# proycon/analiticcl

Hardware: AMD Instinct MI355X
Metric: scored (query,candidate) pairs/sec + queries/sec, 200k-lexicon, len≤16, 1/2/4/8 GPU (higher is better)
Workload: dtype u8

## Files before the change

### analiticcl_amd/csrc/engine.hip

```cpp
#include <hip/hip_runtime.h>

#include <algorithm>
#include <atomic>
#include <functional>
#include <chrono>
#include <cmath>
#include <cstdio>
#include <cstdlib>
#include <cstring>
#include <map>
#include <memory>
#include <mutex>
#include <unordered_map>
#include <numeric>
#include <thread>
#include <type_traits>

#include "engine_internal.h"

namespace anx {

#define HIP_TRY(expr)                                                                          \
  do {                                                                                         \
    hipError_t _e = (expr);                                                                    \
// ... 1043 lines not shown
}
void kernel_timer_enable(bool on) {
  KTimer& t = ktimer();
  std::lock_guard<std::mutex> lk(t.mu);
  ktimer_resolve_locked(t);
  t.acc.clear();
  t.on.store(on);
}
bool kernel_timer_read(const char* name, double* total_ms, uint64_t* launches) {
  KTimer& t = ktimer();
  std::lock_guard<std::mutex> lk(t.mu);
  ktimer_resolve_locked(t);
  auto it = t.acc.find(name ? name : "");
  if (it == t.acc.end()) { if (total_ms) *total_ms = 0.0; if (launches) *launches = 0; return false; }
  if (total_ms) *total_ms = it->second.first;
  if (launches) *launches = it->second.second;
  return true;
}

#include "launch_plan.hpp"

template <int NP>
static void launch_scan(ScanArgs A, uint32_t nadj, uint32_t nbits, uint32_t nsad, hipStream_t st, hipEvent_t e0, hipEvent_t e1) {
  (void)hipEventRecord(e0, st);
  const bool gen = A.want_exact || A.qpairs || !A.drop_len;
  if (nadj) {
    A.ntiles = nadj;
    if (gen) hipLaunchKernelGGL((k_scan_adj<true>), dim3((nadj + 3) / 4), dim3(256), 0, st, A);
    else hipLaunchKernelGGL((k_scan_adj<false>), dim3((nadj + 3) / 4), dim3(256), 0, st, A);
    A.tiles += nadj;
    nbits -= nadj;
  }
  if (nbits) {
    A.ntiles = nbits;
    if (A.want_exact || A.qpairs || !A.drop_len) hipLaunchKernelGGL((k_scan_bits<true>), dim3((nbits + 3) / 4), dim3(256), 0, st, A);
    else hipLaunchKernelGGL((k_scan_bits<false>), dim3((nbits + 3) / 4), dim3(256), 0, st, A);
  }
  (void)hipEventRecord(e1, st);
  if (nsad) {
    A.tiles += nbits;
    A.ntiles = nsad;
    hipLaunchKernelGGL((k_scan_sad<NP>), dim3((nsad + 3) / 4), dim3(256), 0, st, A);
  }
}

static int ensure_raw(Batch* b, size_t slots_per_region, std::string& err) {
  uint32_t shift = 10;
  while (((size_t)1 << shift) < slots_per_region) ++shift;
  if (shift > 25) { err = "pair list exceeds 2^31 slots: split the batch"; return ANX_ELIMIT; }
  const size_t cap = (size_t)SCAN_REGIONS << shift;
  if (cap <= b->raw_cap) return ANX_OK;
  for (void* p : {(void*)b->raw, (void*)b->p_score, (void*)b->p_meta})
    if (p) pool_free(p);
  b->raw = nullptr; b->p_score = nullptr; b->p_meta = nullptr; b->raw_cap = 0;
  int rc;
  if ((rc = dalloc(&b->raw, cap, err))) return rc;
  b->raw_cap = cap;
  b->region_shift = shift;
  return ANX_OK;
}
static int ensure_pair_outputs(Batch* b, std::string& err) {
  if (b->p_meta) return ANX_OK;
  int rc;
  if ((rc = dalloc(&b->p_score, b->raw_cap, err)) || (rc = dalloc(&b->p_meta, b->raw_cap, err))) return rc;
  return ANX_OK;
}
// ... 109 lines not shown

int Run::setup() {
  int rc;
  hints_apply(dl, b);
  if (b->raw_cap == 0 && b->hinted && (rc = ensure_raw(b, (size_t)b->prev_maxfill + (b->prev_maxfill >> 3) + 4096, err))) return rc;
  if (b->raw_cap == 0 && (rc = ensure_raw(b, (nq * (size_t)140 + (size_t)b->ntiles * SCAN_CHUNK) / SCAN_REGIONS / cap_div() + 4096, err)))
    return rc;
  region_cap = 1u << b->region_shift;
  fill_cap = b->prev_maxfill ? (uint32_t)std::min<size_t>(region_cap, (size_t)b->prev_maxfill + (b->prev_maxfill >> 3) + FS_BLK) : region_cap;
  b->fill_cap_launched = fill_cap;
  HIP_TRY(hipEventRecord(b->ev[0], st));
  return ANX_OK;
}

int Run::scan() {
  int rc;
  HIP_TRY(hipMemsetAsync(b->ctl, 0, HR_N * sizeof(uint32_t), st));
  if (b->ntiles == 0) { HIP_TRY(hipEventRecord(b->ev_scan0, st)); HIP_TRY(hipEventRecord(b->ev[5], st)); }
  if (b->ntiles) {
    ScanArgs A = scan_args_of(dl);
    A.tiles = b->d_tiles; A.ntiles = b->ntiles; A.q_bits = b->q_bits; A.q_cv = b->q_cv;
    A.chunk = SCAN_CHUNK;
    A.chunk_fused = switches().scan_chunk_fused ? (uint32_t)switches().scan_chunk_fused : SCAN_CHUNK_FUSED;
#ifdef ANX_DEBUG_SWITCHES
    { const char* e = getenv("ANX_SCAN_CHUNK"); const int v = e ? atoi(e) : 0; if (v >= 32 && v <= 1024) A.chunk = (uint32_t)v; }
#endif
    A.raw = b->raw; A.region_cap = region_cap; A.rctr = b->rctr; A.qexact = b->qexact; A.want_exact = stop;
    A.drop_len = (!stop && !b->keep_all_pairs) ? 1 : 0;
    A.q_rec = b->q_rec;
    A.fuse = (switches().fuse_prefilter && switches().prefilter && A.drop_len) ? 1 : 0;
    A.qpairs = nullptr;
    if (b->count_pairs) {
      if (!b->qpairs && (rc = dalloc(&b->qpairs, nq, err))) return rc;
      HIP_TRY(hipMemsetAsync(b->qpairs, 0, nq * sizeof(uint32_t), st));
      A.qpairs = b->qpairs;
    }
    A.dbg = 0;
#ifdef ANX_DEBUG_SWITCHES
    { const char* e = getenv("ANX_SCAN_DBG"); A.dbg = e ? atoi(e) : 0; }
#endif
    const uint32_t nsad = b->n_sad_tiles, nbits = A.ntiles - nsad, nadj = std::min(b->n_adj_tiles, nbits);
    with_nplanes(dl->nplanes, [&](auto np) { launch_scan<decltype(np)::value>(A, nadj, nbits, nsad, st, b->ev_scan0, b->ev[5]); });
  }
  HIP_TRY(hipEventRecord(b->ev[1], st));
  b->n_raw = (uint32_t)(SCAN_REGIONS << b->region_shift);
  return ANX_OK;
// ... 171 lines not shown
    maxfill = std::max(maxfill, c[RC_RAW]);
    b->region_fill[r] = c[RC_RAW];
    n_slots += c[RC_RAW];
    n_valid += c[RC_VALID];
    n_fused += c[RC_FUSED];
    n_adj_rows += c[RC_ADJ];
    n_adj_rows_first += c[RC_ADJ_FIRST];
    for (int i = 0; i <= NBITPLANES; ++i) {
      uint64_t v;
      memcpy(&v, c + RC_TESTS + 2 * i, sizeof v);
      b->n_tests_kind[i] += v;
      b->n_class_tests += v;
    }
    surv_fill = std::max(surv_fill, h[HR_SCTR + r * RC_STRIDE]);
    nsel += h[HR_SCTR + r * RC_STRIDE + 1];
    for (int l = 0; l < 3; ++l) list_fill = std::max(list_fill, h[HR_LCTR + (l * SCAN_REGIONS + r) * RC_STRIDE]);
  }
  const uint32_t total_surv = h[HR_TOTAL_SURV], total_results = h[HR_TOTAL_RESULTS];
  b->conf_fallback = b->conf_mode != 0 && (h[HR_CONF + 1] != 0 || b->conf_skipped);
  b->stats.n_conf_scripts = b->conf_mode ? h[HR_CONF] : 0;
  b->stats.n_adj_tiles = std::min(b->n_adj_tiles, b->ntiles - b->n_sad_tiles);
  int rc;
  bool again = false;
  if (maxfill > (1u << b->region_shift)) {
    if ((rc = ensure_raw(b, (size_t)maxfill + (maxfill >> 3) + 4096, err))) return rc;
    again = true;
  }
  if (maxfill > b->fill_cap_launched) again = true;
  if ((size_t)surv_fill > b->surv_region_cap) again = true;
  if (list_fill && (size_t)list_fill > b->list_cap) again = true;
  if (!dl->any_variants && (size_t)total_surv > b->surv_cap) {
    if ((rc = ensure_surv(b, (size_t)total_surv + (total_surv >> 2) + 1024, err))) return rc;
    again = true;
  }
  b->prev_maxfill = std::max(b->prev_maxfill, maxfill);
  b->prev_surv_fill = std::max(b->prev_surv_fill, surv_fill);
  b->prev_list_fill = std::max(b->prev_list_fill, list_fill);
  if (again) { *retry = true; b->runs_finished++; return ANX_OK; }
  if (b->runs_finished++ == 0) hints_record(dl, b, maxfill, surv_fill, list_fill, total_surv);
  if (maxfill == 0) b->n_raw = 0;
  b->n_pairs = n_valid - h[HR_CTR + CTR_SKIPPED];
  b->n_surv = total_surv;
  b->n_sel = nsel;
  b->n_results = total_results;
  b->max_rows = h[HR_CTR + CTR_MAXROWS];
  b->ran = true;
  anx_batch_stats& s = b->stats;
  s.n_queries = nq;
  s.n_pairs = b->n_pairs;
  s.n_class_tests = b->n_class_tests;
  s.n_results = total_results;
  s.n_scan_blocks = b->ntiles;
  for (int i = 0; i <= NBITPLANES; ++i) s.n_tests_kind[i] = b->n_tests_kind[i];
  s.n_pair_slots = n_slots;
  s.n_survivors = total_surv;
// ... 656 lines not shown
```

### analiticcl_amd/csrc/host_model.cpp

```cpp
#include "host_model.h"
#include "adjacency.h"

#include <sched.h>
#if defined(__SSE2__)
#include <emmintrin.h>
#endif

#include <thread>

#include <algorithm>
#include <cmath>
#include <cstdio>
#include <cstring>
#include <fstream>
#include <functional>
#include <numeric>
#include <sstream>

#include "unicode_tables.inc"

namespace anx {

static std::vector<uint32_t> make_primes() {
  std::vector<uint32_t> p;
// ... 482 lines not shown
  lexicons.push_back(path);
  return ANX_OK;
}

static int pick_planes(int nsym) {
  const int need = (nsym + 3) / 4;
  for (int v : {8, 16, 24, 32, 42})
    if (need <= v) return v;
  return -1;
}

namespace {
struct SwitchDef { const char* name; void (*set)(Switches&, const char*); };
int flag01(const char* v, int dflt) { return !v ? dflt : (v[0] == '0' ? 0 : 1); }
const SwitchDef kSwitches[] = {
    {"ANX_ENCODE", [](Switches& s, const char* v) { s.encode_host = v && strcmp(v, "host") == 0; }},
    {"ANX_SCAN", [](Switches& s, const char* v) { s.scan_sad = v && strcmp(v, "sad") == 0; }},
    {"ANX_SCAN_WALK", [](Switches& s, const char* v) { s.scan_walk_flat = v && strcmp(v, "flat") == 0; }},
    {"ANX_SCAN_TQ", [](Switches& s, const char* v) { const int x = v ? atoi(v) : 0; s.scan_tq = x >= 1 && x <= 64 ? x : 0; }},
    {"ANX_SCAN_ADJ", [](Switches& s, const char* v) { s.scan_adj = flag01(v, 1); }},
    {"ANX_ADJ_BUILD", [](Switches& s, const char* v) { s.adj_build_host = v && strcmp(v, "host") == 0; }},
    {"ANX_ADJ_CLOSURE", [](Switches& s, const char* v) { const int x = v ? atoi(v) : 2; s.adj_closure = x >= 0 && x <= kAdjMaxClosure ? x : kAdjMaxClosure; }},
    {"ANX_SCAN_CHUNK_FUSED", [](Switches& s, const char* v) { const int x = v ? atoi(v) : 0; s.scan_chunk_fused = x >= 32 && x <= 1024 ? x : 0; }},
    {"ANX_ADJ_FAIL", [](Switches& s, const char* v) { s.adj_fail = flag01(v, 0); }},
    {"ANX_SMALL", [](Switches& s, const char* v) { s.small_path = flag01(v, 1); }},
    {"ANX_SURV_SEG", [](Switches& s, const char* v) { const int x = v ? atoi(v) : 32; s.surv_seg = x >= 0 && x <= 256 ? x : 32; }},
    {"ANX_ENC_PRIORITY", [](Switches& s, const char* v) { s.enc_priority = flag01(v, 1); }},
    {"ANX_HINTS", [](Switches& s, const char* v) { s.hints = flag01(v, 1); }},
    {"ANX_ADJ_MB", [](Switches& s, const char* v) { const long x = v ? atol(v) : 0; s.adj_budget_mb = x > 0 ? x : 16384; }},
    {"ANX_SIG_GROUPS", [](Switches& s, const char* v) { const int x = v ? atoi(v) : 0; s.sig_groups = x >= 1 && x <= 8 ? x : 0; }},
    {"ANX_SIG_SEARCH", [](Switches& s, const char* v) { s.sig_search = flag01(v, 1); }},
    {"ANX_PREFILTER", [](Switches& s, const char* v) { s.prefilter = flag01(v, 1); }},
    {"ANX_SCORE_FAST", [](Switches& s, const char* v) { s.score_fast = flag01(v, 1); }},
    {"ANX_FS_SPLIT", [](Switches& s, const char* v) { s.fs_split = flag01(v, 1); }},
    {"ANX_FS_PLANES", [](Switches& s, const char* v) { s.fs_planes = flag01(v, 1); }},
    {"ANX_FS_B7", [](Switches& s, const char* v) { s.fs_b7 = flag01(v, 1); }},
    {"ANX_SCAN_FUSE", [](Switches& s, const char* v) { s.fuse_prefilter = flag01(v, 1); }},
    {"ANX_CAP_DIV", [](Switches& s, const char* v) { const long x = v ? atol(v) : 0; s.cap_div = x > 1 ? x : 1; }},
    {"ANX_MAX_BATCH", [](Switches& s, const char* v) { const long x = v ? atol(v) : 0; s.max_batch = x > 0 ? x : (4l << 20); }},
    {"ANX_RUN_OVERLAP", [](Switches& s, const char* v) { s.run_overlap = (v && atoi(v) == 0 && v[0] == '0') ? 0 : 1; }},
    {"ANX_SHARD_POLICY", [](Switches& s, const char* v) { s.shard_by_length = (v && strcmp(v, "range") == 0) ? 0 : 1; }},
    {"ANX_SHARD_MIN", [](Switches& s, const char* v) { const long x = v ? atol(v) : 0; s.shard_min = x > 0 ? x : 8192; }},
    {"ANX_CONFUSABLES", [](Switches& s, const char* v) { s.confusables_host = v && strcmp(v, "host") == 0; }},
    {"ANX_LATTICE", [](Switches& s, const char* v) { s.lattice_host = v && strcmp(v, "host") == 0; }},
    {"ANX_SEARCH_ONEPASS", [](Switches& s, const char* v) { s.search_onepass = flag01(v, 1); }},
    {"ANX_ENCODE_TIMING", [](Switches& s, const char* v) { s.encode_timing = v != nullptr && v[0] != 0 && v[0] != '0'; }},
// ... 524 lines not shown
```

### analiticcl_amd/csrc/host_model.h

```cpp
#pragma once
#include <functional>
#include <cstdint>
#include <atomic>
#include <memory>
#include <mutex>
#include <string>
#include <unordered_map>
#include <vector>

#include "../../include/anx.h"
#include "confusables_core.hpp"
#include "contextrules_flat.hpp"

namespace anx {

constexpr int kMaxSymbols = 255;
constexpr int kMaxAlphabet = 166;
constexpr int kMaxAnagramDistance = 12;
constexpr int kMaxEditDistance = 12;

struct AlphabetMember {
  std::string bytes;
  int nchars;
};
// ... 32 lines not shown
  int scan_walk_flat = 0;
  int scan_tq = 0;
  int scan_adj = 1;
  int adj_build_host = 0;
  int adj_closure = 2;
  long adj_budget_mb = 16384;
  int sig_groups = 0;
  int sig_search = 1;
  int prefilter = 1;
  int score_fast = 1;
  int fs_planes = 1;
  int fs_split = 1;
  int fs_b7 = 1;
  int fuse_prefilter = 1;
  long cap_div = 1;
  long max_batch = 4l << 20;
  int run_overlap = 1;
  int shard_by_length = 1;
  long shard_min = 8192;
  int confusables_host = 0;
  int lattice_host = 0;
  int search_onepass = 1;
  int scan_chunk_fused = 0;
  int adj_fail = 0;
  int small_path = 1;
  int enc_priority = 1;
  int hints = 1;
  int encode_timing = 0;
  int search_timing = 0;
  int search_parts = 4;
  long search_parts_min = 2l << 20;
  long search_part_bytes = 4l << 20;
  int search_prio = 1;
  int search_early_output = 1;
  int search_first_pct = 50;
  int surv_seg = 32;
  int learn_fold_host = 0;
  int learn_hash_bits = 63;
};
Switches& switches();
bool set_switch(const char* name, const char* value);

struct VariantRef {
  bool variant_of;
  uint64_t id;
  double score;
// ... 178 lines not shown
```

### analiticcl_amd/csrc/kernels_common.hpp

```cpp
#pragma once

struct Tile {
  uint32_t q0, nq;
  uint32_t s0, s1;
  uint32_t k;
  uint32_t lq;
  uint32_t sig_lo, sig_hi;
  uint32_t kind;
  uint32_t d;
  uint32_t kend;
  uint32_t ball0, balln;
  uint32_t adj;
  uint32_t flags;
};
constexpr uint32_t BALL_MAX = 4096;
constexpr uint32_t SIG_BYTE_MAX = 120;

constexpr int kSymbolPlanesMaxA = 61;
__host__ __device__ inline void symbol_planes16(const uint8_t* row, uint32_t len, uint32_t (&w)[3]) {
  uint32_t p[6] = {0u, 0u, 0u, 0u, 0u, 0u};
  for (uint32_t i = 0; i < 16u && i < len; ++i) {
    const uint32_t v = (uint32_t)row[i] + 1u;
    for (uint32_t b = 0; b < 6u; ++b) p[b] |= ((v >> b) & 1u) << i;
  }
  w[0] = p[0] | p[1] << 16; w[1] = p[2] | p[3] << 16; w[2] = p[4] | p[5] << 16;
}

constexpr int NBITPLANES = 4;
constexpr uint32_t SCAN_TQ = 64;
constexpr uint32_t SCAN_TQ_DEFAULT = 48;
constexpr uint32_t SCAN_HITS = 512;
constexpr uint32_t SCAN_MASKW = 2048;
constexpr uint32_t SCAN_PBUF = 128;
constexpr uint32_t SCAN_CHUNK = 256;
constexpr uint32_t SCAN_CHUNK_FUSED = 128;
constexpr uint32_t SCAN_REGIONS = 64;
constexpr uint32_t RC_STRIDE = 32;
constexpr uint32_t RAW_INVALID = 0xFFFFFFFFu;
constexpr uint32_t RAW_ENTRY_MASK = 0x3FFFFFFFu;
constexpr uint32_t RAW_PREFILTERED = 0x40000000u;
constexpr uint32_t META_SKIPPED = 0xFFFFFFFFu;

struct EntRec {
  uint32_t vocab, freq, order, meta;
};

struct DevAlphabet {
  int16_t* fast = nullptr;
  uint32_t* coff = nullptr;
  uint4* cand = nullptr;
  uint8_t* bytes = nullptr;
  uint8_t* sym_group = nullptr;
  uint2* lower = nullptr;
  uint32_t nlower = 0;
  uint32_t* siglen_begin = nullptr;
};

struct BatchShell {
// ... 191 lines not shown
```

### analiticcl_amd/csrc/kernels_scan.hpp

```cpp
#pragma once

enum { RC_RAW = 0, RC_VALID = 1, RC_FUSED = 2 , RC_TESTS = 4 ,
       RC_ADJ = 14 , RC_ADJ_FIRST = 15  };

struct WaveOut {
  uint32_t base, left;
  uint32_t emitted;
  uint32_t nbase;
  uint32_t split;
  uint32_t rbase, rend;
  uint32_t* ctr;
  uint32_t chunk;
};
__device__ inline uint32_t wave_inclusive_scan(uint32_t x) {
  uint32_t v = x;
  v += (uint32_t)__builtin_amdgcn_update_dpp(0, (int)x, 0x111, 0xF, 0xF, false);
  v += (uint32_t)__builtin_amdgcn_update_dpp(0, (int)x, 0x112, 0xF, 0xF, false);
  v += (uint32_t)__builtin_amdgcn_update_dpp(0, (int)x, 0x113, 0xF, 0xF, false);
  v += (uint32_t)__builtin_amdgcn_update_dpp(0, (int)v, 0x114, 0xF, 0xE, false);
  v += (uint32_t)__builtin_amdgcn_update_dpp(0, (int)v, 0x118, 0xF, 0xC, false);
  v += (uint32_t)__builtin_amdgcn_update_dpp(0, (int)v, 0x142, 0xA, 0xF, false);
  v += (uint32_t)__builtin_amdgcn_update_dpp(0, (int)v, 0x143, 0xC, 0xF, false);
  return v;
}
__device__ inline uint32_t wave_reserve(WaveOut& w, uint32_t ntot, uint32_t lane, uint32_t* total_out) {
  const uint32_t incl = wave_inclusive_scan(ntot);
  const uint32_t total = (uint32_t)__builtin_amdgcn_readlane((int)incl, 63);
  *total_out = total;
  w.split = w.left;
  if (total > w.left) {
    const uint32_t rest = total - w.left;
    const uint32_t need = rest > w.chunk ? rest : w.chunk;
    uint32_t b = 0;
    if (lane == 0) b = atomicAdd(&w.ctr[RC_RAW], need);
    w.nbase = w.rbase + __shfl(b, 0);
  }
  return incl - ntot;
}
__device__ inline void wave_reserve_total(WaveOut& w, uint32_t total, uint32_t lane) {
  w.split = w.left;
  if (total > w.left) {
    const uint32_t rest = total - w.left;
    const uint32_t need = rest > w.chunk ? rest : w.chunk;
    uint32_t b = 0;
    if (lane == 0) b = atomicAdd(&w.ctr[RC_RAW], need);
    w.nbase = w.rbase + (uint32_t)__builtin_amdgcn_readfirstlane((int)b);
  }
}
__device__ inline uint32_t wave_slot(const WaveOut& w, uint32_t g) {
  return g < w.split ? w.base + g : w.nbase + (g - w.split);
}
__device__ inline void wave_commit(WaveOut& w, uint32_t total) {
  if (total > w.left) {
    const uint32_t rest = total - w.left;
    const uint32_t need = rest > w.chunk ? rest : w.chunk;
    w.base = w.nbase + rest;
    w.left = need - rest;
  } else {
    w.base += total;
    w.left -= total;
  }
  w.emitted += total;
}
__device__ inline void wave_close(const WaveOut& w, uint32_t lane, uint2* __restrict__ raw) {
  for (uint32_t i = lane; i < w.left; i += 64)
    if (w.base + i < w.rend) raw[w.base + i] = make_uint2(RAW_INVALID, 0u);
  if (lane == 0 && w.emitted) atomicAdd(&w.ctr[RC_VALID], w.emitted);
}

struct ScanArgs {
  const Tile* tiles;
  uint32_t ntiles;
  const uint32_t* q_bits;
  const uint32_t* q_cv;
  const uint32_t* cls_bits;
  const uint32_t* cls_planes;
  const uint4* scan_rec;
  const uint2* scan_rec34;
  uint32_t pad_rec;
  uint32_t cstride;
  uint32_t pad_class;
  const uint8_t* cls_len;
  const uint32_t* cls_off;
  const uint4* sig;
  const uint4* sig_e;
  const uint4* sighash;
  const uint4* sighash_e;
  uint32_t hash_mask;
  const unsigned long long* ball;
  const uint32_t* adj_hdr;
  const uint2* adj_planes;
  const uint32_t* adj_ids;
  const uint32_t* sig_cbeg;
  uint2* raw;
  uint32_t region_cap;
  uint32_t chunk;
  uint32_t chunk_fused;
  uint32_t* rctr;
  const uint32_t* qexact;
  int want_exact;
  int drop_len;
  const uint4* q_rec;
  const uint4* e_rec;
  int fuse;
  uint32_t* qpairs;
  int dbg;
};

__device__ inline int32_t bcnt_acc(uint32_t x, int32_t acc) {
  int32_t r;
  asm("v_bcnt_u32_b32 %0, %1, %2" : "=v"(r) : "v"(x), "v"(acc));
  return r;
}
__device__ inline int32_t bcnt_acc_s(uint32_t x, int32_t acc) {
  int32_t r;
  asm("v_bcnt_u32_b32 %0, %1, %2" : "=v"(r) : "v"(x), "s"(acc));
  return r;
}

template <bool BITS, int NP, bool GEN, bool ADJ = false>
__device__ inline void scan_tile(const ScanArgs& AA, const Tile& t, uint32_t item, uint32_t* __restrict__ stage, uint32_t* __restrict__ hits,
                                 uint32_t* __restrict__ qlds, uint4* __restrict__ qsym, uint32_t* __restrict__ pbuf) {
  ScanArgs A = AA;
  if (!GEN) { A.want_exact = 0; A.qpairs = nullptr; A.drop_len = 1; A.qexact = nullptr; }
  constexpr int CPL = BITS ? 4 : (NP <= 8 ? 4 : NP <= 16 ? 2 : 1);
  constexpr int W = BITS ? NBITPLANES : NP;
  constexpr int QSTRIDE = BITS ? NBITPLANES : NP;
  constexpr uint32_t CHUNK = 64u * CPL;
  const uint32_t lane = threadIdx.x & 63;
  const uint32_t* __restrict__ cls_words = BITS ? A.cls_bits : A.cls_planes;
  const uint8_t* __restrict__ cls_len = A.cls_len;
  const uint32_t* __restrict__ cls_off = A.cls_off;
  uint2* __restrict__ raw = A.raw;
  const uint32_t cstride = A.cstride;
  const uint32_t region = item % SCAN_REGIONS;
  WaveOut wo{0, 0, 0, 0, 0, region * A.region_cap, (region + 1) * A.region_cap, A.rctr + region * RC_STRIDE, A.chunk};
  uint32_t ns = 0;
  uint32_t nchunks = 0;
  uint32_t arend = 0;
  int32_t alc[4] = {0, 0, 0, 0};
  uint2 apl[4] = {};
  uint32_t aid[4] = {};
  auto adj_load = [&](uint32_t row, uint2 (&pl)[4], uint32_t (&id)[4]) {
#pragma unroll
    for (int j = 0; j < 4; ++j) {
      pl[j] = make_uint2(0u, 0u);
      id[j] = A.pad_rec;
      if (row + (uint32_t)j < arend) {
        const size_t p = (size_t)(row + (uint32_t)j) * 64u + lane;
        pl[j] = A.adj_planes[p];
        id[j] = A.adj_ids[p];
      }
    }
  };
  {
    const uint32_t* __restrict__ src = (BITS ? A.q_bits : A.q_cv) + (size_t)t.q0 * QSTRIDE;
    for (uint32_t i = lane; i < t.nq * QSTRIDE; i += 64) qlds[i] = src[i];
  }
  const bool fuse = BITS && A.fuse && t.lq <= 16u && t.d <= 3u;
  if (fuse) wo.chunk = A.chunk_fused;
  if (BITS && fuse && lane < t.nq) qsym[lane] = rec32(A.q_rec, t.q0 + lane)[0];
  constexpr uint32_t PBUF = SCAN_PBUF;
  uint32_t nfused = 0;
  uint32_t npb = 0, phead = 0;

  uint32_t nhits = 0;
  uint32_t counted_only = 0;
  auto emit_dense = [&](bool fin) {
    while (npb >= 64u || (fin && npb)) {
      const uint32_t cnt = npb < 64u ? npb : 64u;
      const bool act = lane < cnt;
      const uint32_t pr = pbuf[(phead + lane) & (PBUF - 1u)];
      const uint32_t e = act ? (pr & 0x3FFFFFFu) : 0u, ql = act ? (pr >> 26) : 0u;
      bool keep = act;
      uint32_t flag = 0u;
      if (ANX_DBG(A.dbg) & 16) keep = false;
      if (BITS && fuse && !(ANX_DBG(A.dbg) & 16)) {
        nfused += cnt;
        const uint4 C = rec32(A.e_rec, e)[0];
        const int lc = (int)(rec32(A.e_rec, e)[1].x & 0xFFu), lq = (int)t.lq, d = (int)t.d;
        const uint4 Q = qsym[ql];
        const bool filt = act && lc <= 16;
        const int ml = lq > lc ? lq : lc;
// ... 18 lines not shown
      if (total) {
        wave_reserve_total(wo, total, lane);
        if (keep) {
          const uint32_t q = t.q0 + ql;
          uint32_t exact = 0u;
          if (A.want_exact) exact = A.qexact[q] == A.scan_rec[e].w ? 0x80000000u : 0u;
          const uint32_t g = __builtin_amdgcn_mbcnt_hi((uint32_t)(km >> 32), __builtin_amdgcn_mbcnt_lo((uint32_t)km, 0u));
          const uint32_t pos = wave_slot(wo, g);
          if (pos < wo.rend) raw[pos] = make_uint2(q, e | exact | flag);
        }
        wave_commit(wo, total);
      }
      phead = (phead + cnt) & (PBUF - 1u);
      npb -= cnt;
    }
  };
  auto flush = [&]() {
    for (uint32_t r0 = 0; r0 < nhits; r0 += 64) {
      const uint32_t idx = r0 + lane;
      uint32_t c = 0, m = 0, e0 = 0, ne = 0, qb = 0;
      if (idx < nhits) {
        bool count_only;
        if (BITS) {
          const uint32_t hx = reinterpret_cast<const uint16_t*>(hits + SCAN_HITS)[idx];
          m = hits[idx];
          qb = ((hx >> 8) & 1u) << 5;
          count_only = (hx >> 9) & 1u;
          e0 = stage[hx & 0xFFu];
          ne = 1;
          c = A.qpairs ? A.scan_rec[e0].w : 0u;
        } else {
          c = hits[2 * idx];
          m = hits[2 * idx + 1];
          qb = ((c >> 27) & 1u) << 5;
          c &= (1u << 27) - 1u;
          const uint32_t lc = cls_len[c];
          e0 = cls_off[c];
          ne = cls_off[c + 1] - e0;
          const uint32_t diff = lc > t.lq ? lc - t.lq : t.lq - lc;
          count_only = A.drop_len && diff > t.d;
        }
        if (A.qpairs) {
          for (uint32_t mm = m; mm; mm &= mm - 1u) {
            const uint32_t q = t.q0 + qb + (uint32_t)__ffs((int)mm) - 1u;
            if (!A.want_exact || A.qexact[q] == 0xFFFFFFFFu || A.qexact[q] == c) atomicAdd(&A.qpairs[q], ne);
          }
        }
        if (count_only) {
          counted_only += (uint32_t)__popc(m) * ne;
          m = 0;
        }
// ... 22 lines not shown
          m &= m - 1u;
          const uint32_t q = t.q0 + qb + bit;
          const uint32_t exact = (A.want_exact && A.qexact[q] == c) ? 0x80000000u : 0u;
          for (uint32_t i = 0; i < ne; ++i, ++g) dst[g] = make_uint2(q, (e0 + i) | exact);
        }
      } else {
        while (m) {
          const uint32_t bit = (uint32_t)__ffs((int)m) - 1u;
          m &= m - 1u;
          const uint32_t q = t.q0 + qb + bit;
          const uint32_t exact = (A.want_exact && A.qexact[q] == c) ? 0x80000000u : 0u;
          for (uint32_t i = 0; i < ne; ++i, ++g) {
            const uint32_t pos = wave_slot(wo, g);
            if (pos < wo.rend) raw[pos] = make_uint2(q, (e0 + i) | exact);
          }
        }
      }
      wave_commit(wo, total);
    }
    nhits = 0;
  };

  auto process = [&]() {
    ++nchunks;
    if (ANX_DBG(A.dbg) & 2) return;
    uint32_t cid[CPL], cw[CPL][W];
    int32_t thr[CPL];
    const bool need34 = BITS && ((t.kend >> 8) & 0xFFu) < t.nq;
#pragma unroll
    for (int j = 0; j < CPL; ++j) {
      const uint32_t idx = (uint32_t)j * 64u + lane;
      int32_t lc;
      if (ADJ) {
        const uint2 pl = apl[j];
        const uint32_t id = aid[j];
        stage[idx] = id;
        uint2 hi = make_uint2(0u, 0u);
        if (need34) hi = A.scan_rec34[id];
        cw[j][0] = pl.x; cw[j][1] = pl.y;
        if (W > 2) { cw[j][2] = hi.x; cw[j][W - 1] = hi.y; }
        lc = alc[j];
        const int32_t diff = lc > (int32_t)t.lq ? lc - (int32_t)t.lq : (int32_t)t.lq - lc;
        cid[j] = (A.drop_len && diff > (int32_t)t.d) ? id | (1u << 28) : id;
      } else {
      cid[j] = idx < ns ? stage[idx] : (BITS ? A.pad_rec : A.pad_class);
      if (BITS) {
        const uint4 mt = A.scan_rec[cid[j]];
        uint2 hi = make_uint2(0u, 0u);
        if (need34) hi = A.scan_rec34[cid[j]];
        const uint32_t plw[4] = {mt.x, mt.y, hi.x, hi.y};
#pragma unroll
        for (int p = 0; p < W; ++p) cw[j][p] = plw[p];
        lc = (int32_t)mt.z;
        const int32_t diff = lc > (int32_t)t.lq ? lc - (int32_t)t.lq : (int32_t)t.lq - lc;
        if (A.drop_len && diff > (int32_t)t.d) cid[j] |= 1u << 28;
      } else {
#pragma unroll
        for (int p = 0; p < W; ++p) cw[j][p] = cls_words[(size_t)p * cstride + cid[j]];
        lc = (int32_t)cls_len[cid[j]];
      }
      }
      if (BITS) {
        const int32_t need = ((int32_t)t.lq - (int32_t)t.k + lc + 1) >> 1;
        thr[j] = -(need < 1 ? 1 : need);
      } else {
// ... 31 lines not shown
        uint32_t qi = lo;
        for (; qi + 2 <= hi; qi += 2) {
          test_query(tw, qi);
          test_query(tw, qi + 1);
        }
        if (qi < hi) test_query(tw, qi);
      };
      if (BITS) {
        const uint32_t pend = qb + npass;
        auto clampr = [&](uint32_t x) { return (x < qb ? qb : (x > pend ? pend : x)) - qb; };
        const uint32_t b1 = clampr(t.kend & 0xFFu), b2 = clampr((t.kend >> 8) & 0xFFu), b3 = clampr((t.kend >> 16) & 0xFFu);
        run_queries(std::integral_constant<int, 1>{}, 0u, b1);
        run_queries(std::integral_constant<int, 2>{}, b1, b2);
        run_queries(std::integral_constant<int, 3>{}, b2, b3);
        run_queries(std::integral_constant<int, BITS ? 4 : 1>{}, b3, npass);
      } else {
        run_queries(std::integral_constant<int, BITS ? 1 : NP>{}, 0u, npass);
      }
      const uint32_t valid = npass >= 32u ? 0xFFFFFFFFu : ((1u << npass) - 1u);
      uint32_t any = 0;
#pragma unroll
      for (int j = 0; j < CPL; ++j) {
        hm[j] = ~hm[j] & valid;
        any |= hm[j];
      }
      if (__ballot(any != 0) == 0ull || (ANX_DBG(A.dbg) & 8)) continue;
#pragma unroll
      for (int j = 0; j < CPL; ++j) {
        const bool nz = hm[j] != 0;
        const unsigned long long bm = __ballot(nz);
        const uint32_t cnt = (uint32_t)__popcll(bm);
        if (cnt) {
          if (nz) {
            const uint32_t pos = nhits + __builtin_amdgcn_mbcnt_hi((uint32_t)(bm >> 32), __builtin_amdgcn_mbcnt_lo((uint32_t)bm, 0u));
            const uint32_t hmask = __brev(hm[j]) >> (32u - npass);
            if (BITS) {
              hits[pos] = hmask;
              reinterpret_cast<uint16_t*>(hits + SCAN_HITS)[pos] = (uint16_t)(((uint32_t)j * 64u + lane) | ((qb >> 5) << 8) | (((cid[j] >> 28) & 1u) << 9));
            } else {
              hits[2 * pos] = cid[j] | ((qb >> 5) << 27);
              hits[2 * pos + 1] = hmask;
            }
          }
          nhits += cnt;
        }
      }
      if (!BITS && nhits > SCAN_HITS - CHUNK) flush();
    }
    if (BITS) flush();
  };

  uint32_t* __restrict__ sdelta = stage + CHUNK;
  uint32_t* __restrict__ smask = stage + CHUNK + 64;
  auto stage_runs = [&](bool ok, uint32_t cb, uint32_t n) {
    ok = ok && n != 0u;
    const unsigned long long okm = __ballot(ok);
    if (!okm || (ANX_DBG(A.dbg) & 4)) return;
    const uint32_t cnt = ok ? n : 0u;
    const uint32_t incl = wave_inclusive_scan(cnt);
    const uint32_t carry = ns & 63u;
    const uint32_t total = carry + (uint32_t)__builtin_amdgcn_readlane((int)incl, 63);
    uint32_t wbase = ns - carry;
    const uint32_t endp = carry + incl - 1u;
    if (ok) sdelta[__builtin_amdgcn_mbcnt_hi((uint32_t)(okm >> 32), __builtin_amdgcn_mbcnt_lo((uint32_t)okm, 0u))] = cb + cnt - 1u - endp;
    uint32_t rbase = 0;
    for (uint32_t w0 = 0; w0 < total; w0 += SCAN_MASKW) {
      if (lane < SCAN_MASKW / 32u) smask[lane] = 0u;
      if (ok && endp - w0 < SCAN_MASKW) atomicOr(smask + ((endp - w0) >> 5), 1u << (endp & 31u));
      const uint32_t wend = total < w0 + SCAN_MASKW ? total : w0 + SCAN_MASKW;
      for (uint32_t p0 = w0; p0 < wend; p0 += 64) {
        const uint32_t mlo = (uint32_t)__builtin_amdgcn_readfirstlane((int)smask[((p0 - w0) >> 6) * 2u]), mhi = (uint32_t)__builtin_amdgcn_readfirstlane((int)smask[((p0 - w0) >> 6) * 2u + 1u]);
        const uint32_t r = rbase + __builtin_amdgcn_mbcnt_hi(mhi, __builtin_amdgcn_mbcnt_lo(mlo, 0u));
        rbase += (uint32_t)__popc(mlo) + (uint32_t)__popc(mhi);
        const uint32_t p = p0 + lane;
        const uint32_t id = sdelta[r & 63u] + p;
        if (p >= carry && p < total) stage[wbase + lane] = id;
        if (p0 + 64u <= total) {
          wbase += 64u;
          ns = wbase;
          if (wbase == CHUNK) {
            process();
            ns = 0;
            wbase = 0;
          }
        } else {
          ns = wbase + (total - p0);
        }
      }
    }
  };
  const uint4* __restrict__ sigtab = BITS ? A.sig_e : A.sig;
  if (ADJ) {
    const cptr_u32 hp = (cptr_u32)(A.adj_hdr + (size_t)(t.adj - 1u) * 8u);
    const uint32_t row0 = hp[0], c0 = hp[1], c1 = hp[2], c2 = hp[3], c3 = hp[4], c4 = hp[5], c5 = hp[6], c6 = hp[7];
    uint32_t rbeg = t.k >= 3u ? 0u : t.k == 2u ? c0 : t.k == 1u ? c1 : c2;
    uint32_t rend = t.k >= 3u ? c6 : t.k == 2u ? c5 : t.k == 1u ? c4 : c3;
    if (t.flags & 2u) { rbeg = t.s0; rend = t.s1; }
    arend = row0 + rend;
    if (lane == 0 && rend > rbeg) {
      atomicAdd(&wo.ctr[RC_ADJ], rend - rbeg);
      if (t.flags & 1u) atomicAdd(&wo.ctr[RC_ADJ_FIRST], rend - rbeg);
    }
    uint2 npl[4];
    uint32_t nid[4];
    if (rbeg < rend) adj_load(row0 + rbeg, npl, nid);
    for (uint32_t r = rbeg; r < rend; r += (uint32_t)CPL) {
#pragma unroll
      for (int j = 0; j < 4; ++j) {
        const uint32_t rr = r + (uint32_t)j;
        alc[j] = (int32_t)t.lq - 3 + (int32_t)((rr >= c0) + (rr >= c1) + (rr >= c2) + (rr >= c3) + (rr >= c4) + (rr >= c5));
        apl[j] = npl[j];
        aid[j] = nid[j];
      }
      if (r + (uint32_t)CPL < rend) adj_load(row0 + r + (uint32_t)CPL, npl, nid);
      process();
    }
  } else if (t.balln) {
    const unsigned long long H = 0x8080808080808080ull;
    const unsigned long long sq = (unsigned long long)t.sig_lo | (unsigned long long)t.sig_hi << 32;
    const uint4* __restrict__ htab = BITS ? A.sighash_e : A.sighash;
    for (uint32_t base = 0; base < t.balln; base += 64) {
      const uint32_t i = base + lane;
      bool found = false;
      uint32_t first = 0, count = 0;
      if (i < t.balln) {
// ... 12 lines not shown
      }
      stage_runs(found, first, count);
    }
  } else {
    const uint4* __restrict__ sigp = sigtab + t.s0 + lane;
    uint4 sg_next = t.s0 < t.s1 ? *sigp : make_uint4(0xFFFFFFFFu, 0xFFFFFFFFu, 0u, 0u);
    for (uint32_t sb = t.s0; sb < t.s1; sb += 64) {
      const uint4 sg = sg_next;
      sigp += 64;
      if (sb + 64 < t.s1) sg_next = *sigp;
      const bool ok = __builtin_amdgcn_sad_u8(sg.x, t.sig_lo, __builtin_amdgcn_sad_u8(sg.y, t.sig_hi, 0u)) <= t.k;
      stage_runs(ok, sg.z, sg.w);
    }
  }
  if (!ADJ && ns) process();
  flush();
  if (BITS) emit_dense(true);
  if (A.drop_len) {
    const uint32_t tot = (uint32_t)__builtin_amdgcn_readlane((int)wave_inclusive_scan(counted_only), 63);
    wo.emitted += tot;
  }
  wave_close(wo, lane, raw);
  if (BITS && lane == 0 && nfused) atomicAdd(&wo.ctr[RC_FUSED], nfused);
  if (lane == 0 && nchunks) {
    if (BITS) {
      const uint32_t e[5] = {0u, t.kend & 0xFFu, (t.kend >> 8) & 0xFFu, (t.kend >> 16) & 0xFFu, t.nq};
      for (int k = 1; k <= NBITPLANES; ++k)
        if (e[k] > e[k - 1])
          atomicAdd(reinterpret_cast<unsigned long long*>(wo.ctr + RC_TESTS + 2 * k), (unsigned long long)nchunks * CHUNK * (e[k] - e[k - 1]));
    } else {
      atomicAdd(reinterpret_cast<unsigned long long*>(wo.ctr + RC_TESTS), (unsigned long long)nchunks * CHUNK * t.nq);
    }
  }
}

constexpr uint32_t SCAN_STAGE = 64 * 4 + 64 + SCAN_MASKW / 32;
template <int NP, bool BITS, bool GEN, bool ADJ = false>
__device__ inline void scan_wave(const ScanArgs& A) {
  constexpr int QWORDS = SCAN_TQ * (BITS ? NBITPLANES : NP);
  __shared__ uint32_t s_qlds[4][QWORDS];
  __shared__ __attribute__((aligned(16))) uint32_t s_stage[4][ADJ ? 64 * 4 : SCAN_STAGE];
  __shared__ uint32_t s_hits[4][BITS ? SCAN_HITS + SCAN_HITS / 2 : 2 * SCAN_HITS];
  __shared__ uint4 s_qsym[BITS ? 4 : 1][BITS ? SCAN_TQ : 1];
  __shared__ uint32_t s_pbuf[BITS ? 4 : 1][BITS ? SCAN_PBUF : 1];
  const uint32_t wid = threadIdx.x >> 6;
  const uint32_t item = (uint32_t)__builtin_amdgcn_readfirstlane((int)(blockIdx.x * 4u + wid));
  if (item >= A.ntiles) return;
  const cptr_u32 tp = (cptr_u32)(A.tiles + item);
  Tile t;
  t.q0 = tp[0]; t.nq = tp[1]; t.s0 = tp[2]; t.s1 = tp[3]; t.k = tp[4]; t.lq = tp[5]; t.sig_lo = tp[6]; t.sig_hi = tp[7]; t.kind = tp[8]; t.d = tp[9]; t.kend = tp[10]; t.ball0 = tp[11]; t.balln = tp[12]; t.adj = tp[13]; t.flags = tp[14];
  scan_tile<BITS, NP, GEN, ADJ>(A, t, item, s_stage[wid], s_hits[wid], s_qlds[wid], s_qsym[BITS ? wid : 0], s_pbuf[BITS ? wid : 0]);
}
template <bool GEN>
__global__ __launch_bounds__(256) __attribute__((amdgpu_waves_per_eu(5, 8))) void k_scan_bits(ScanArgs A) { scan_wave<8, true, GEN>(A); }
template <bool GEN>
__global__ __launch_bounds__(256) __attribute__((amdgpu_waves_per_eu(6, 8))) void k_scan_adj(ScanArgs A) { scan_wave<8, true, GEN, true>(A); }
template <int NP>
__global__ __launch_bounds__(256) void k_scan_sad(ScanArgs A) { scan_wave<NP, false, true>(A); }


template <int NP>
__global__ __launch_bounds__(256) void k_scan_small(ScanArgs A) {
  constexpr int QW = NP > NBITPLANES ? NP : NBITPLANES;
  __shared__ uint32_t s_qlds[4][QW];
  __shared__ __attribute__((aligned(16))) uint32_t s_stage[4][SCAN_STAGE];
  __shared__ uint32_t s_hits[4][2 * SCAN_HITS];
  __shared__ uint4 s_qsym[4][1];
  __shared__ uint32_t s_pbuf[4][SCAN_PBUF];
  const uint32_t wid = threadIdx.x >> 6;
  const uint32_t item = (uint32_t)__builtin_amdgcn_readfirstlane((int)(blockIdx.x * 4u + wid));
  if (item >= A.ntiles) return;
  const cptr_u32 tp = (cptr_u32)(A.tiles + item);
  Tile t;
  t.q0 = tp[0]; t.nq = tp[1]; t.s0 = tp[2]; t.s1 = tp[3]; t.k = tp[4]; t.lq = tp[5]; t.sig_lo = tp[6]; t.sig_hi = tp[7]; t.kind = tp[8]; t.d = tp[9]; t.kend = tp[10]; t.ball0 = tp[11]; t.balln = tp[12]; t.adj = tp[13]; t.flags = tp[14];
// ... 6 lines not shown
```

### analiticcl_amd/csrc/small_path.hpp

```cpp
#pragma once

constexpr uint32_t SMALL_MAX_BYTES = 64;
constexpr uint32_t SMALL_SHIFT = 15;
constexpr uint32_t SMALL_SURV_CAP = 16384;
constexpr uint32_t SMALL_LIST_BLOCKS = 2;
constexpr uint32_t SMALL_FS_BLK = 512;
constexpr uint32_t SMALL_FETCH_BLOCKS = 8;
constexpr uint32_t SMALL_ROWS_PER_Q = 16;
constexpr uint32_t SMALL_CF_BLOCKS = 160;

struct SmallCtx {
  int device = 0;
  hipStream_t st = nullptr;
  char* h_in = nullptr;
  char* h_out = nullptr;
  SmallEnc enc;
  uint32_t *counters = nullptr, *rctr = nullptr, *sctr = nullptr, *lctr = nullptr, *qsurv = nullptr, *soff = nullptr, *qcur = nullptr, *qmaxfreq = nullptr, *qexpand = nullptr,
           *r_count = nullptr;
  uint2* raw = nullptr;
  SurvRec* surv = nullptr;
  uint32_t *list8 = nullptr, *listg = nullptr, *listw = nullptr;
  SurvRow* c_rows = nullptr;
  DevRow* r_rows = nullptr;
  double* t_key = nullptr;
// ... 154 lines not shown
  } guard{rows, st, false};
  if (!host_result_is_pinned(rows)) return 1;
  SmallCtl* h_ctl = reinterpret_cast<SmallCtl*>(c->h_out);
  unsigned long long* h_off64 = reinterpret_cast<unsigned long long*>(c->h_out + 64);
  h_ctl->rows = 0xFFFFFFFEu;
  SmallZero z{};
  {
    uint32_t* zp[8] = {c->counters, c->rctr, c->sctr, c->lctr, c->qsurv, c->qmaxfreq, c->qexpand, conf_mode ? c->cf.ctr : nullptr};
    const uint32_t zn[8] = {CTR_N, SCAN_REGIONS * RC_STRIDE, SCAN_REGIONS * RC_STRIDE, 3 * SCAN_REGIONS * RC_STRIDE, n32, n32, n32, conf_mode ? 8u : 0u};
    for (int i = 0; i < 8; ++i) { z.p[i] = zp[i]; z.n[i] = zn[i]; }
  }
  const uint8_t* in_blob = reinterpret_cast<const uint8_t*>(c->h_in);
  const uint32_t* in_off = h_off;
  const uint32_t slots = n32 <= 128u ? 32u : n32 <= 512u ? 16u : 8u;
  guard.drain = true;
  SmallEnc enc = c->enc;
  if (!conf_mode) enc.text = nullptr, enc.textoff = nullptr;
  int rc = small_encode_launch(m, dl, enc, in_blob, in_off, n32, qw, p, z, slots, true, h_off, st, err);
  if (rc) return rc;
  const uint32_t region_cap = 1u << SMALL_SHIFT;
  {
    ScanArgs A = scan_args_of(dl);
    A.tiles = c->enc.tiles; A.ntiles = slots * n32; A.q_bits = c->enc.q_bits; A.q_cv = c->enc.q_cv;
    A.chunk = 64; A.chunk_fused = 32;
    A.raw = c->raw; A.region_cap = region_cap; A.rctr = c->rctr; A.qexact = c->enc.qexact; A.want_exact = 0; A.drop_len = 1;
    A.q_rec = c->enc.q_rec;
    A.fuse = (switches().fuse_prefilter && switches().prefilter) ? 1 : 0;
    A.qpairs = nullptr; A.dbg = 0;
    const dim3 grid((A.ntiles + 3) / 4);
    with_nplanes(dl->nplanes, [&](auto np) { hipLaunchKernelGGL(k_scan_small<decltype(np)::value>, grid, dim3(256), 0, st, A); });
  }
  ScorePlan plan = score_plan_of(m, dl, p.score_threshold, qw, d);
  plan.sa.dbg = 0; plan.sa.store_pairs = 0;
  if (!plan.fits()) return 1;
  const ScoreArgs& sa = plan.sa;
  const uint32_t threads = plan.threads;
  const int fastD = plan.fastD;
  const SurvOut so{c->surv, c->sctr, SMALL_SURV_CAP, nullptr, 0u};
  const SlotLists sl = slot_lists_of(c->list8, c->listg, c->listw, c->lctr, SMALL_SURV_CAP);
  const PairArgs pa = pair_args_of(dl, c->raw, c->enc.q_meta, c->enc.q_rows, c->enc.q_rec, nullptr, nullptr, c->qmaxfreq, c->qsurv, c->qexpand);
  uint32_t fs_cap = 2048;
  while (fs_cap < region_cap && fs_cap < n32 * 12u + 2048u) fs_cap *= 2u;
  FilterArgs fa;
  fa.region_shift = SMALL_SHIFT; fa.rctr = c->rctr; fa.qexact = c->enc.qexact; fa.stop = 0; fa.enable = plan.enable_filter;
  const bool use8 = fastD > 0 && threads == 256;
  fa.use_nw8 = (plan.have_long_q || use8) ? 1 : 0; fa.counters = c->counters; fa.stat_ctr = c->sctr; fa.fill_cap = fs_cap; fa.blk = SMALL_FS_BLK;
  {
// ... 65 lines not shown
```

Before: 56.04 billion.

## Grow scan output chunks geometrically, skip count-only adjacency rows, widen hit records

The scan kernel's per-wave output reservation now starts at a small first chunk and doubles up to the fused cap, which cuts wasted raw-buffer slots and lowers region fill. Adjacency tiles that only need counting (the length difference exceeds the distance) now just count their hits and skip hit emission, and the final flush is skipped when the hit buffer has room. The stage LDS buffer is dropped for adjacency tiles because hit records now carry the full 26-bit candidate id, and test counting is moved to per-row-range for adjacency tiles. The retry logic scales survivor and list estimates by the overflow ratio so buffers grow in one step instead of several retries. A kernel timer is also added around the scan launches.

Result: faster. 56.93 billion, median of 6 (+1.6%).

```diff
diff --git a/analiticcl_amd/csrc/engine.hip b/analiticcl_amd/csrc/engine.hip
--- a/analiticcl_amd/csrc/engine.hip
+++ b/analiticcl_amd/csrc/engine.hip
@@ -1089,6 +1089,7 @@
 
 template <int NP>
 static void launch_scan(ScanArgs A, uint32_t nadj, uint32_t nbits, uint32_t nsad, hipStream_t st, hipEvent_t e0, hipEvent_t e1) {
+  const int kt = ktimer_begin("k_scan", st);
   (void)hipEventRecord(e0, st);
   const bool gen = A.want_exact || A.qpairs || !A.drop_len;
   if (nadj) {
@@ -1109,6 +1110,7 @@
     A.ntiles = nsad;
     hipLaunchKernelGGL((k_scan_sad<NP>), dim3((nsad + 3) / 4), dim3(256), 0, st, A);
   }
+  ktimer_end(kt, st);
 }
 
 static int ensure_raw(Batch* b, size_t slots_per_region, std::string& err) {
@@ -1264,6 +1266,7 @@
     A.tiles = b->d_tiles; A.ntiles = b->ntiles; A.q_bits = b->q_bits; A.q_cv = b->q_cv;
     A.chunk = SCAN_CHUNK;
     A.chunk_fused = switches().scan_chunk_fused ? (uint32_t)switches().scan_chunk_fused : SCAN_CHUNK_FUSED;
+    A.chunk_first = switches().scan_chunk_first ? (uint32_t)switches().scan_chunk_first : SCAN_CHUNK_FIRST;
 #ifdef ANX_DEBUG_SWITCHES
     { const char* e = getenv("ANX_SCAN_CHUNK"); const int v = e ? atoi(e) : 0; if (v >= 32 && v <= 1024) A.chunk = (uint32_t)v; }
 #endif
@@ -1481,6 +1484,16 @@
   b->stats.n_adj_tiles = std::min(b->n_adj_tiles, b->ntiles - b->n_sad_tiles);
   int rc;
   bool again = false;
+  size_t surv_need = total_surv;
+  {
+    const uint32_t covered = std::min(1u << b->region_shift, b->fill_cap_launched);
+    if (maxfill > covered && covered) {
+      const double f = (double)maxfill / covered;
+      surv_fill = (uint32_t)std::min(surv_fill * f, 4.0e9);
+      list_fill = (uint32_t)std::min(list_fill * f, 4.0e9);
+      surv_need = (size_t)(total_surv * f);
+    }
+  }
   if (maxfill > (1u << b->region_shift)) {
     if ((rc = ensure_raw(b, (size_t)maxfill + (maxfill >> 3) + 4096, err))) return rc;
     again = true;
@@ -1488,8 +1501,8 @@
   if (maxfill > b->fill_cap_launched) again = true;
   if ((size_t)surv_fill > b->surv_region_cap) again = true;
   if (list_fill && (size_t)list_fill > b->list_cap) again = true;
-  if (!dl->any_variants && (size_t)total_surv > b->surv_cap) {
-    if ((rc = ensure_surv(b, (size_t)total_surv + (total_surv >> 2) + 1024, err))) return rc;
+  if (!dl->any_variants && surv_need > b->surv_cap) {
+    if ((rc = ensure_surv(b, surv_need + (surv_need >> 2) + 1024, err))) return rc;
     again = true;
   }
   b->prev_maxfill = std::max(b->prev_maxfill, maxfill);
diff --git a/analiticcl_amd/csrc/host_model.cpp b/analiticcl_amd/csrc/host_model.cpp
--- a/analiticcl_amd/csrc/host_model.cpp
+++ b/analiticcl_amd/csrc/host_model.cpp
@@ -528,6 +528,7 @@
     {"ANX_ADJ_BUILD", [](Switches& s, const char* v) { s.adj_build_host = v && strcmp(v, "host") == 0; }},
     {"ANX_ADJ_CLOSURE", [](Switches& s, const char* v) { const int x = v ? atoi(v) : 2; s.adj_closure = x >= 0 && x <= kAdjMaxClosure ? x : kAdjMaxClosure; }},
     {"ANX_SCAN_CHUNK_FUSED", [](Switches& s, const char* v) { const int x = v ? atoi(v) : 0; s.scan_chunk_fused = x >= 32 && x <= 1024 ? x : 0; }},
+    {"ANX_SCAN_CHUNK_FIRST", [](Switches& s, const char* v) { const int x = v ? atoi(v) : 0; s.scan_chunk_first = x >= 32 && x <= 1024 ? x / 32 * 32 : 0; }},
     {"ANX_ADJ_FAIL", [](Switches& s, const char* v) { s.adj_fail = flag01(v, 0); }},
     {"ANX_SMALL", [](Switches& s, const char* v) { s.small_path = flag01(v, 1); }},
     {"ANX_SURV_SEG", [](Switches& s, const char* v) { const int x = v ? atoi(v) : 32; s.surv_seg = x >= 0 && x <= 256 ? x : 32; }},
diff --git a/analiticcl_amd/csrc/host_model.h b/analiticcl_amd/csrc/host_model.h
--- a/analiticcl_amd/csrc/host_model.h
+++ b/analiticcl_amd/csrc/host_model.h
@@ -78,6 +78,7 @@
   int lattice_host = 0;
   int search_onepass = 1;
   int scan_chunk_fused = 0;
+  int scan_chunk_first = 0;
   int adj_fail = 0;
   int small_path = 1;
   int enc_priority = 1;
diff --git a/analiticcl_amd/csrc/kernels_common.hpp b/analiticcl_amd/csrc/kernels_common.hpp
--- a/analiticcl_amd/csrc/kernels_common.hpp
+++ b/analiticcl_amd/csrc/kernels_common.hpp
@@ -34,6 +34,7 @@
 constexpr uint32_t SCAN_PBUF = 128;
 constexpr uint32_t SCAN_CHUNK = 256;
 constexpr uint32_t SCAN_CHUNK_FUSED = 128;
+constexpr uint32_t SCAN_CHUNK_FIRST = 32;
 constexpr uint32_t SCAN_REGIONS = 64;
 constexpr uint32_t RC_STRIDE = 32;
 constexpr uint32_t RAW_INVALID = 0xFFFFFFFFu;
diff --git a/analiticcl_amd/csrc/kernels_scan.hpp b/analiticcl_amd/csrc/kernels_scan.hpp
--- a/analiticcl_amd/csrc/kernels_scan.hpp
+++ b/analiticcl_amd/csrc/kernels_scan.hpp
@@ -10,8 +10,9 @@
   uint32_t split;
   uint32_t rbase, rend;
   uint32_t* ctr;
-  uint32_t chunk;
+  uint32_t sizes;
 };
+__device__ inline uint32_t wave_sizes(uint32_t first, uint32_t cap) { return (first < cap ? first : cap) | cap << 16; }
 __device__ inline uint32_t wave_inclusive_scan(uint32_t x) {
   uint32_t v = x;
   v += (uint32_t)__builtin_amdgcn_update_dpp(0, (int)x, 0x111, 0xF, 0xF, false);
@@ -30,7 +31,7 @@
   w.split = w.left;
   if (total > w.left) {
     const uint32_t rest = total - w.left;
-    const uint32_t need = rest > w.chunk ? rest : w.chunk;
+    const uint32_t size = w.sizes & 0xFFFFu, need = rest > size ? rest : size;
     uint32_t b = 0;
     if (lane == 0) b = atomicAdd(&w.ctr[RC_RAW], need);
     w.nbase = w.rbase + __shfl(b, 0);
@@ -41,7 +42,7 @@
   w.split = w.left;
   if (total > w.left) {
     const uint32_t rest = total - w.left;
-    const uint32_t need = rest > w.chunk ? rest : w.chunk;
+    const uint32_t size = w.sizes & 0xFFFFu, need = rest > size ? rest : size;
     uint32_t b = 0;
     if (lane == 0) b = atomicAdd(&w.ctr[RC_RAW], need);
     w.nbase = w.rbase + (uint32_t)__builtin_amdgcn_readfirstlane((int)b);
@@ -53,9 +54,11 @@
 __device__ inline void wave_commit(WaveOut& w, uint32_t total) {
   if (total > w.left) {
     const uint32_t rest = total - w.left;
-    const uint32_t need = rest > w.chunk ? rest : w.chunk;
+    const uint32_t size = w.sizes & 0xFFFFu, need = rest > size ? rest : size;
     w.base = w.nbase + rest;
     w.left = need - rest;
+    const uint32_t cap = w.sizes >> 16;
+    w.sizes = (size * 2u < cap ? size * 2u : cap) | cap << 16;
   } else {
     w.base += total;
     w.left -= total;
@@ -96,6 +99,7 @@
   uint32_t region_cap;
   uint32_t chunk;
   uint32_t chunk_fused;
+  uint32_t chunk_first;
   uint32_t* rctr;
   const uint32_t* qexact;
   int want_exact;
@@ -134,7 +138,7 @@
   uint2* __restrict__ raw = A.raw;
   const uint32_t cstride = A.cstride;
   const uint32_t region = item % SCAN_REGIONS;
-  WaveOut wo{0, 0, 0, 0, 0, region * A.region_cap, (region + 1) * A.region_cap, A.rctr + region * RC_STRIDE, A.chunk};
+  WaveOut wo{0, 0, 0, 0, 0, region * A.region_cap, (region + 1) * A.region_cap, A.rctr + region * RC_STRIDE, 0};
   uint32_t ns = 0;
   uint32_t nchunks = 0;
   uint32_t arend = 0;
@@ -158,7 +162,7 @@
     for (uint32_t i = lane; i < t.nq * QSTRIDE; i += 64) qlds[i] = src[i];
   }
   const bool fuse = BITS && A.fuse && t.lq <= 16u && t.d <= 3u;
-  if (fuse) wo.chunk = A.chunk_fused;
+  wo.sizes = fuse ? wave_sizes(A.chunk_first, A.chunk_fused) : wave_sizes(A.chunk, A.chunk);
   if (BITS && fuse && lane < t.nq) qsym[lane] = rec32(A.q_rec, t.q0 + lane)[0];
   constexpr uint32_t PBUF = SCAN_PBUF;
   uint32_t nfused = 0;
@@ -223,11 +227,11 @@
       if (idx < nhits) {
         bool count_only;
         if (BITS) {
-          const uint32_t hx = reinterpret_cast<const uint16_t*>(hits + SCAN_HITS)[idx];
+          const uint32_t hx = hits[SCAN_HITS + idx];
           m = hits[idx];
-          qb = ((hx >> 8) & 1u) << 5;
-          count_only = (hx >> 9) & 1u;
-          e0 = stage[hx & 0xFFu];
+          qb = ((hx >> 26) & 1u) << 5;
+          count_only = (hx >> 27) & 1u;
+          e0 = hx & 0x3FFFFFFu;
           ne = 1;
           c = A.qpairs ? A.scan_rec[e0].w : 0u;
         } else {
@@ -296,10 +300,13 @@
   };
 
   auto process = [&]() {
-    ++nchunks;
+    if (!ADJ) ++nchunks;
     if (ANX_DBG(A.dbg) & 2) return;
     uint32_t cid[CPL], cw[CPL][W];
     int32_t thr[CPL];
+    constexpr bool ROWCOUNT = ADJ && !GEN;
+    bool conly[CPL] = {};
+    bool all_conly = ROWCOUNT;
     const bool need34 = BITS && ((t.kend >> 8) & 0xFFu) < t.nq;
 #pragma unroll
     for (int j = 0; j < CPL; ++j) {
@@ -308,13 +315,14 @@
       if (ADJ) {
         const uint2 pl = apl[j];
         const uint32_t id = aid[j];
-        stage[idx] = id;
         uint2 hi = make_uint2(0u, 0u);
         if (need34) hi = A.scan_rec34[id];
         cw[j][0] = pl.x; cw[j][1] = pl.y;
         if (W > 2) { cw[j][2] = hi.x; cw[j][W - 1] = hi.y; }
         lc = alc[j];
         const int32_t diff = lc > (int32_t)t.lq ? lc - (int32_t)t.lq : (int32_t)t.lq - lc;
+        conly[j] = ROWCOUNT && diff > (int32_t)t.d && !(ANX_DBG(A.dbg) & 64);
+        all_conly = all_conly && conly[j];
         cid[j] = (A.drop_len && diff > (int32_t)t.d) ? id | (1u << 28) : id;
       } else {
       cid[j] = idx < ns ? stage[idx] : (BITS ? A.pad_rec : A.pad_class);
@@ -392,8 +400,13 @@
 #pragma unroll
       for (int j = 0; j < CPL; ++j) {
         hm[j] = ~hm[j] & valid;
+        if (ADJ && conly[j]) {
+          counted_only += (uint32_t)__popc(hm[j]);
+          hm[j] = 0u;
+        }
         any |= hm[j];
       }
+      if (ADJ && all_conly) continue;
       if (__ballot(any != 0) == 0ull || (ANX_DBG(A.dbg) & 8)) continue;
 #pragma unroll
       for (int j = 0; j < CPL; ++j) {
@@ -406,7 +419,7 @@
             const uint32_t hmask = __brev(hm[j]) >> (32u - npass);
             if (BITS) {
               hits[pos] = hmask;
-              reinterpret_cast<uint16_t*>(hits + SCAN_HITS)[pos] = (uint16_t)(((uint32_t)j * 64u + lane) | ((qb >> 5) << 8) | (((cid[j] >> 28) & 1u) << 9));
+              hits[SCAN_HITS + pos] = (cid[j] & 0x3FFFFFFu) | ((qb >> 5) << 26) | (((cid[j] >> 28) & 1u) << 27);
             } else {
               hits[2 * pos] = cid[j] | ((qb >> 5) << 27);
               hits[2 * pos + 1] = hmask;
@@ -417,7 +430,7 @@
       }
       if (!BITS && nhits > SCAN_HITS - CHUNK) flush();
     }
-    if (BITS) flush();
+    if (BITS && (GEN || nhits + ((t.nq + 31u) >> 5) * CHUNK > SCAN_HITS || (ANX_DBG(A.dbg) & 128))) flush();
   };
 
   uint32_t* __restrict__ sdelta = stage + CHUNK;
@@ -460,6 +473,17 @@
     }
   };
   const uint4* __restrict__ sigtab = BITS ? A.sig_e : A.sig;
+  auto count_tests = [&](uint32_t nch) {
+    if (lane != 0 || nch == 0u) return;
+    if (BITS) {
+      const uint32_t e[5] = {0u, t.kend & 0xFFu, (t.kend >> 8) & 0xFFu, (t.kend >> 16) & 0xFFu, t.nq};
+      for (int k = 1; k <= NBITPLANES; ++k)
+        if (e[k] > e[k - 1])
+          atomicAdd(reinterpret_cast<unsigned long long*>(wo.ctr + RC_TESTS + 2 * k), (unsigned long long)nch * CHUNK * (e[k] - e[k - 1]));
+    } else {
+      atomicAdd(reinterpret_cast<unsigned long long*>(wo.ctr + RC_TESTS), (unsigned long long)nch * CHUNK * t.nq);
+    }
+  };
   if (ADJ) {
     const cptr_u32 hp = (cptr_u32)(A.adj_hdr + (size_t)(t.adj - 1u) * 8u);
     const uint32_t row0 = hp[0], c0 = hp[1], c1 = hp[2], c2 = hp[3], c3 = hp[4], c4 = hp[5], c5 = hp[6], c6 = hp[7];
@@ -471,6 +495,7 @@
       atomicAdd(&wo.ctr[RC_ADJ], rend - rbeg);
       if (t.flags & 1u) atomicAdd(&wo.ctr[RC_ADJ_FIRST], rend - rbeg);
     }
+    if (rend > rbeg) count_tests((rend - rbeg + (uint32_t)CPL - 1u) / (uint32_t)CPL);
     uint2 npl[4];
     uint32_t nid[4];
     if (rbeg < rend) adj_load(row0 + rbeg, npl, nid);
@@ -529,16 +554,7 @@
   }
   wave_close(wo, lane, raw);
   if (BITS && lane == 0 && nfused) atomicAdd(&wo.ctr[RC_FUSED], nfused);
-  if (lane == 0 && nchunks) {
-    if (BITS) {
-      const uint32_t e[5] = {0u, t.kend & 0xFFu, (t.kend >> 8) & 0xFFu, (t.kend >> 16) & 0xFFu, t.nq};
-      for (int k = 1; k <= NBITPLANES; ++k)
-        if (e[k] > e[k - 1])
-          atomicAdd(reinterpret_cast<unsigned long long*>(wo.ctr + RC_TESTS + 2 * k), (unsigned long long)nchunks * CHUNK * (e[k] - e[k - 1]));
-    } else {
-      atomicAdd(reinterpret_cast<unsigned long long*>(wo.ctr + RC_TESTS), (unsigned long long)nchunks * CHUNK * t.nq);
-    }
-  }
+  if (!ADJ) count_tests(nchunks);
 }
 
 constexpr uint32_t SCAN_STAGE = 64 * 4 + 64 + SCAN_MASKW / 32;
@@ -546,8 +562,12 @@
 __device__ inline void scan_wave(const ScanArgs& A) {
   constexpr int QWORDS = SCAN_TQ * (BITS ? NBITPLANES : NP);
   __shared__ uint32_t s_qlds[4][QWORDS];
-  __shared__ __attribute__((aligned(16))) uint32_t s_stage[4][ADJ ? 64 * 4 : SCAN_STAGE];
-  __shared__ uint32_t s_hits[4][BITS ? SCAN_HITS + SCAN_HITS / 2 : 2 * SCAN_HITS];
+  uint32_t* stage = nullptr;
+  if constexpr (!ADJ) {
+    __shared__ __attribute__((aligned(16))) uint32_t s_stage[4][SCAN_STAGE];
+    stage = s_stage[threadIdx.x >> 6];
+  }
+  __shared__ uint32_t s_hits[4][2 * SCAN_HITS];
   __shared__ uint4 s_qsym[BITS ? 4 : 1][BITS ? SCAN_TQ : 1];
   __shared__ uint32_t s_pbuf[BITS ? 4 : 1][BITS ? SCAN_PBUF : 1];
   const uint32_t wid = threadIdx.x >> 6;
@@ -556,7 +576,7 @@
   const cptr_u32 tp = (cptr_u32)(A.tiles + item);
   Tile t;
   t.q0 = tp[0]; t.nq = tp[1]; t.s0 = tp[2]; t.s1 = tp[3]; t.k = tp[4]; t.lq = tp[5]; t.sig_lo = tp[6]; t.sig_hi = tp[7]; t.kind = tp[8]; t.d = tp[9]; t.kend = tp[10]; t.ball0 = tp[11]; t.balln = tp[12]; t.adj = tp[13]; t.flags = tp[14];
-  scan_tile<BITS, NP, GEN, ADJ>(A, t, item, s_stage[wid], s_hits[wid], s_qlds[wid], s_qsym[BITS ? wid : 0], s_pbuf[BITS ? wid : 0]);
+  scan_tile<BITS, NP, GEN, ADJ>(A, t, item, stage, s_hits[wid], s_qlds[wid], s_qsym[BITS ? wid : 0], s_pbuf[BITS ? wid : 0]);
 }
 template <bool GEN>
 __global__ __launch_bounds__(256) __attribute__((amdgpu_waves_per_eu(5, 8))) void k_scan_bits(ScanArgs A) { scan_wave<8, true, GEN>(A); }
diff --git a/analiticcl_amd/csrc/small_path.hpp b/analiticcl_amd/csrc/small_path.hpp
--- a/analiticcl_amd/csrc/small_path.hpp
+++ b/analiticcl_amd/csrc/small_path.hpp
@@ -200,7 +200,7 @@
   {
     ScanArgs A = scan_args_of(dl);
     A.tiles = c->enc.tiles; A.ntiles = slots * n32; A.q_bits = c->enc.q_bits; A.q_cv = c->enc.q_cv;
-    A.chunk = 64; A.chunk_fused = 32;
+    A.chunk = 64; A.chunk_fused = 32; A.chunk_first = 64;
     A.raw = c->raw; A.region_cap = region_cap; A.rctr = c->rctr; A.qexact = c->enc.qexact; A.want_exact = 0; A.drop_len = 1;
     A.q_rec = c->enc.q_rec;
     A.fuse = (switches().fuse_prefilter && switches().prefilter) ? 1 : 0;
```
